# hasindu2008/cornetto

Measured on AMD Instinct MI355X. Metric: Gbases/s scanned (telowin+sdust+boringbits), higher is better.
Workload: dtype u8/u16 integer

## Files before the change

cornetto_amd/csrc/common.hpp:

```cpp
#pragma once
#include <hip/hip_runtime.h>

#include <cstdarg>
#include <cstdint>
#include <cstdio>
#include <cstdlib>
#include <cstring>
#include <algorithm>
#include <atomic>
#include <string>
#include <utility>
#include <vector>

#include "../../include/cornetto_accel.h"

#ifndef CN_STREAM_PRIO
#define CN_STREAM_PRIO 3
#endif

inline std::atomic<uint64_t> cn_uid_counter{1};

struct cornetto_accel {
    int device = 0;
    std::string tf_lut_key;
// ... 23 lines not shown
    int sd_slots = 0;
    int sd_cus = 0;
    int sift_per_cu = 0;
    int sift_per_cu_default = -1;
    int lazy = 0;
    hipStream_t copy_stream = nullptr;
    hipEvent_t ev_cp = nullptr;
    bool copies_pending = false;
    volatile int boost = 0;
    volatile unsigned long long launch_seq = 0;
    hipEvent_t ev3 = nullptr;
    int share = 100;
    int sd_stats = 0;
    struct SdPend {
        int state = 0;
        const void *a = nullptr;
        int32_t T = 0, W = 0;
        void *of = nullptr;
        size_t m_cap = 0, n_cap = 0, cap = 0;
        int64_t key = 0, n_done = 0;
        bool walk_pending = false;
    } sd_pend;
    unsigned long long sd_last[256] = {0};
    uint32_t scan_epoch = 0, scan_tickets = 0;
    uint32_t st_epoch = 0, st_tickets = 0;
    int timing = 2;
};

static inline void *cn_ws(cornetto_accel_t *h, int slot, size_t bytes)
{
    cornetto_accel::Ws &w = h->dev[slot];
    if (bytes == 0) bytes = 16;
    if (w.bytes >= bytes) return w.p;
#ifdef CN_WS_ASYNC
    if (w.p) (void)hipFreeAsync(w.p, h->stream);
    w.p = nullptr;
    w.bytes = 0;
    const size_t want = bytes + bytes / 8;
    if (hipMallocAsync(&w.p, want, h->stream) == hipSuccess) w.bytes = want;
    else w.p = nullptr;
    return w.p;
#else
    if (w.p) (void)hipFree(w.p);
    w.p = nullptr;
    w.bytes = 0;
    const size_t want = bytes + bytes / 8;
// ... 292 lines not shown
```

cornetto_amd/csrc/ivlmerge.hpp:

```cpp
#pragma once
#include "common.hpp"
#include "scan.hpp"

namespace cnivl {
namespace {

constexpr int ST_THREADS = 256, ST_ITEMS = 4, ST_TILE = ST_THREADS * ST_ITEMS;

__device__ __forceinline__ unsigned long long st_shfl_up(unsigned long long v, int d)
{
    return ((unsigned long long)(unsigned)__shfl_up((int)(v >> 32), d) << 32) | (unsigned)__shfl_up((int)v, d);
}

__global__ __launch_bounds__(ST_THREADS) void st_local(const cornetto_ivl_t *v, int64_t n, unsigned long long *kprev, unsigned long long *tile_max)
{
    __shared__ unsigned long long wmax[ST_THREADS / 64];
    const int t = threadIdx.x, lane = t & 63, wv = t >> 6;
    const int64_t j0 = (int64_t)blockIdx.x * ST_TILE + (int64_t)t * ST_ITEMS;
    unsigned long long k[ST_ITEMS], run = 0;
#pragma unroll
    for (int i = 0; i < ST_ITEMS; ++i) {
        k[i] = 0;
        if (j0 + i < n) k[i] = ((unsigned long long)(unsigned)v[j0 + i].ctg << 32) | (unsigned)v[j0 + i].finish;
        run = k[i] > run ? k[i] : run;
// ... 63 lines not shown
__global__ void st_emit(const cornetto_ivl_t *v, int64_t n, const unsigned long long *kinc, const uint32_t *head, const uint32_t *rank, cornetto_ivl_t *out)
{
    const int64_t j = (int64_t)blockIdx.x * blockDim.x + threadIdx.x;
    if (j >= n) return;
    const uint32_t hd = head[j];
    const uint32_t g = rank[j] + hd - 1u;
    if (hd) {
        out[g].ctg = v[j].ctg;
        out[g].start = v[j].start;
    }
    if (j == n - 1 || head[j + 1]) out[g].finish = (int32_t)(kinc[j] & 0xFFFFFFFFull);
}

struct StArgs {
    const cornetto_ivl_t *v;
    const unsigned long long *d_n;
    int64_t n_cap;
    int32_t dist;
    unsigned long long *st;
    uint32_t *ticket;
    uint32_t ticket_base, epoch;
    cornetto_ivl_t *out;
    unsigned long long *d_count;
};

__device__ __forceinline__ unsigned long long st_wave_max(unsigned long long v)
{
#pragma unroll
    for (int d = 32; d >= 1; d >>= 1) {
        const unsigned long long o = ((unsigned long long)(unsigned)__shfl_xor((int)(v >> 32), d) << 32) | (unsigned)__shfl_xor((int)v, d);
        v = o > v ? o : v;
    }
    return v;
}

__global__ __launch_bounds__(ST_THREADS) void st_fused(StArgs A)
{
    __shared__ unsigned long long wmax[ST_THREADS / 64];
    __shared__ uint32_t wcnt[ST_THREADS / 64];
    __shared__ unsigned long long s_in;
    __shared__ uint32_t s_tile, s_base;
    const int t = threadIdx.x, lane = t & 63, wv = t >> 6;
    if (t == 0) s_tile = atomicAdd(A.ticket, 1u) - A.ticket_base;
    __syncthreads();
    const int64_t tile = s_tile;
    if (tile >= (A.n_cap + ST_TILE - 1) / ST_TILE) return;
    const int64_t n = (int64_t)__hip_atomic_load(A.d_n, __ATOMIC_RELAXED, __HIP_MEMORY_SCOPE_AGENT);
    if (n > A.n_cap) return;
    if (tile * ST_TILE >= n) return;
    const int64_t j0 = tile * ST_TILE + (int64_t)t * ST_ITEMS;
    cornetto_ivl_t x[ST_ITEMS + 1];
    unsigned long long k[ST_ITEMS], run = 0;
#pragma unroll
    for (int i = 0; i <= ST_ITEMS; ++i) {
        x[i] = cornetto_ivl_t{0, 0, 0};
        if (j0 + i < n) x[i] = A.v[j0 + i];
    }
#pragma unroll
    for (int i = 0; i < ST_ITEMS; ++i) {
        k[i] = j0 + i < n ? ((unsigned long long)(unsigned)x[i].ctg << 32) | (unsigned)x[i].finish : 0ull;
        run = k[i] > run ? k[i] : run;
    }
    unsigned long long inc = run;
#pragma unroll
    for (int d = 1; d < 64; d <<= 1) {
        const unsigned long long o = st_shfl_up(inc, d);
        if (lane >= d && o > inc) inc = o;
    }
    if (lane == 63) wmax[wv] = inc;
    __syncthreads();
// ... 79 lines not shown
                for (;;) {
                    c = idx >= 0 ? __hip_atomic_load(&st[4 * idx + 3], __ATOMIC_RELAXED, __HIP_MEMORY_SCOPE_AGENT) : ((2ull << 62) | ctag);
                    const bool ready = (c >> 62) != 0 && (c & (0x3FFFFFFFull << 32)) == ctag;
                    if (__builtin_amdgcn_ballot_w64(!ready) == 0) break;
                    __builtin_amdgcn_s_sleep(1);
                }
                const unsigned long long incl = __builtin_amdgcn_ballot_w64((c >> 62) == 2);
                const uint32_t val = (uint32_t)c;
                if (incl) {
                    const int first = __builtin_ctzll(incl);
                    excl += cnscan::wave_sum(lane <= first ? val : 0u);
                    break;
                }
                excl += cnscan::wave_sum(val);
            }
        }
        if (lane == 0) {
            __hip_atomic_store(&st[4 * tile + 3], (2ull << 62) | ctag | (excl + tcnt), __ATOMIC_RELAXED, __HIP_MEMORY_SCOPE_AGENT);
            s_base = excl;
            if (tile == (n - 1) / ST_TILE && A.d_count) *A.d_count = (unsigned long long)excl + tcnt;
        }
    }
    __syncthreads();
    uint32_t rank = s_base + pre;
#pragma unroll
    for (int i = 0; i < ST_ITEMS; ++i) {
        if (j0 + i >= n) break;
        const uint32_t g = rank + hd[i] - 1u;
        if (hd[i]) {
            A.out[g].ctg = x[i].ctg;
            A.out[g].start = x[i].start;
        }
        if (j0 + i == n - 1 || hd[i + 1]) A.out[g].finish = (int32_t)(kinc[i] & 0xFFFFFFFFull);
        rank += hd[i];
    }
}

static inline int merge_fused(cornetto_accel_t *h, const char *name, const cornetto_ivl_t *d_in, const unsigned long long *d_n, int64_t n_cap, int32_t dist,
                              cornetto_ivl_t *d_out, unsigned long long *d_count)
{
    if (n_cap <= 0) return CORNETTO_OK;
    const int64_t nt = (n_cap + ST_TILE - 1) / ST_TILE;
    const size_t need = 64 + (size_t)nt * 32;
    const bool fresh = h->dev[WS_STITCH].bytes < need;
    uint8_t *ws = (uint8_t *)cn_ws(h, WS_STITCH, need);
    if (!ws) return cn_fail(h, CORNETTO_E_NOMEM, "merge: workspace allocation failed");
    const int rc = [&]() -> int {
        if (fresh) {
            CN_HIP(h, hipMemsetAsync(ws, 0, h->dev[WS_STITCH].bytes, h->stream));
            h->st_tickets = 0;
            h->st_epoch = 0;
        }
        uint32_t epoch = (h->st_epoch + 1) & 0x3FFFFFFFu;
        if (epoch == 0) epoch = 1;
        StArgs A{d_in, d_n, n_cap, dist, reinterpret_cast<unsigned long long *>(ws + 64), reinterpret_cast<uint32_t *>(ws), h->st_tickets, epoch, d_out, d_count};
        CN_LAUNCH(h, name, st_fused<<<dim3((unsigned)nt), dim3(ST_THREADS), 0, h->stream>>>(A));
        h->st_epoch = epoch;
        h->st_tickets += (uint32_t)nt;
        return CORNETTO_OK;
    }();
    if (rc != CORNETTO_OK) h->dev[WS_STITCH].bytes = 0;
    return rc;
}

static inline size_t ws_bytes(size_t n)
{
    const size_t nt = (n + ST_TILE - 1) / ST_TILE;
    return n * 16 + (nt + 1) * 8 + ((n + 4095) / 4096 + 1) * 4 + 64;
}

static inline int merge(cornetto_accel_t *h, const char *name, const cornetto_ivl_t *d_in, int64_t n_in, int32_t dist, uint8_t *ws,
                        cornetto_ivl_t *d_out, unsigned long long *d_count)
{
    if (n_in <= 0) return CORNETTO_OK;
    const size_t n = (size_t)n_in, nt = (n + ST_TILE - 1) / ST_TILE;
    unsigned long long *d_k = (unsigned long long *)ws, *d_tile = d_k + n;
    uint32_t *d_head = (uint32_t *)(d_tile + nt + 1), *d_rank = d_head + n, *d_hp = d_rank + n;
    const unsigned nbn = (unsigned)((n + 255) / 256);
// ... 11 lines not shown
```

cornetto_amd/csrc/scan.hpp:

```cpp
#pragma once
#include "common.hpp"

namespace cnscan {
namespace {

constexpr int SC_THREADS = 256;
constexpr int SC_ITEMS = 16;
constexpr int SC_TILE = SC_THREADS * SC_ITEMS;

__device__ __forceinline__ uint32_t wave_incl(uint32_t v, int lane)
{
#pragma unroll
    for (int d = 1; d < 64; d <<= 1) {
        uint32_t o = __shfl_up(v, d);
        if (lane >= d) v += o;
    }
    return v;
}

__global__ __launch_bounds__(SC_THREADS) void scan_local(const uint32_t *in, int64_t n, int stride, uint32_t *out, uint32_t *partial)
{
    __shared__ uint32_t wtot[SC_THREADS / 64];
    const int t = threadIdx.x, lane = t & 63, wv = t >> 6;
    const int64_t base = (int64_t)blockIdx.x * SC_TILE + (int64_t)t * SC_ITEMS;
// ... 123 lines not shown
        const int64_t i = base + k;
        if (i < n) out[i] += add;
    }
}

struct LbArgs {
    const uint32_t *in;
    int64_t n, np;
    int stride, m;
    Outs4 outs;
    unsigned long long *state;
    uint32_t *ticket;
    uint32_t ticket_base, epoch;
    unsigned long long *total;
};

__device__ __forceinline__ uint32_t wave_sum(uint32_t v)
{
#pragma unroll
    for (int d = 32; d >= 1; d >>= 1) v += __shfl_xor(v, d);
    return v;
}

__global__ __launch_bounds__(SC_THREADS) void scan_lookback(LbArgs A)
{
    __shared__ uint32_t wtot[SC_THREADS / 64];
    __shared__ uint32_t s_gid, s_excl;
    const int t = threadIdx.x, lane = t & 63, wv = t >> 6;
    if (t == 0) s_gid = atomicAdd(A.ticket, 1u) - A.ticket_base;
    __syncthreads();
    const int64_t gid = s_gid;
    if (gid >= (int64_t)A.m * A.np) return;
    const int q = (int)(gid / A.np);
    const int64_t tile = gid - (int64_t)q * A.np;
    const int64_t base = tile * SC_TILE + (int64_t)t * SC_ITEMS;
    uint32_t *const out = A.outs.o[q];
    uint32_t v[SC_ITEMS], s = 0;
#pragma unroll
    for (int k = 0; k < SC_ITEMS; ++k) {
        const int64_t i = base + k;
        v[k] = i < A.n ? A.in[i * A.stride + q] : 0u;
        s += v[k];
    }
    const uint32_t inc = wave_incl(s, lane);
    if (lane == 63) wtot[wv] = inc;
    __syncthreads();
    uint32_t pre = inc - s, bt = 0;
#pragma unroll
    for (int w = 0; w < SC_THREADS / 64; ++w) {
        if (w < wv) pre += wtot[w];
        bt += wtot[w];
    }
    if (wv == 0) {
        unsigned long long *const st = A.state + (int64_t)q * A.np;
        const unsigned long long tag = (unsigned long long)(A.epoch & 0x3FFFFFFFu) << 32;
        uint32_t excl = 0;
        if (tile > 0) {
            if (lane == 0) __hip_atomic_store(&st[tile], (1ull << 62) | tag | bt, __ATOMIC_RELAXED, __HIP_MEMORY_SCOPE_AGENT);
            for (int64_t pos = tile - 1;; pos -= 64) {
                const int64_t idx = pos - lane;
                unsigned long long x;
                for (;;) {
                    x = idx >= 0 ? __hip_atomic_load(&st[idx], __ATOMIC_RELAXED, __HIP_MEMORY_SCOPE_AGENT) : ((2ull << 62) | tag);
                    const bool ready = (x >> 62) != 0 && (x & (0x3FFFFFFFull << 32)) == tag;
                    if (__builtin_amdgcn_ballot_w64(!ready) == 0) break;
                    __builtin_amdgcn_s_sleep(1);
                }
                const unsigned long long incl = __builtin_amdgcn_ballot_w64((x >> 62) == 2);
                uint32_t val = (uint32_t)x;
                if (incl) {
                    const int first = __builtin_ctzll(incl);
                    excl += wave_sum(lane <= first ? val : 0u);
                    break;
                }
                excl += wave_sum(val);
            }
        }
        if (lane == 0) {
            __hip_atomic_store(&st[tile], (2ull << 62) | tag | (excl + bt), __ATOMIC_RELAXED, __HIP_MEMORY_SCOPE_AGENT);
            s_excl = excl;
            if (A.total && tile == A.np - 1) A.total[q] = (unsigned long long)excl + bt;
        }
    }
    __syncthreads();
    pre += s_excl;
#pragma unroll
    for (int k = 0; k < SC_ITEMS; ++k) {
        const int64_t i = base + k;
        if (i < A.n) out[i] = pre;
        pre += v[k];
    }
}

static inline int scan_mode()
{
    static const int mode = CN_DEV_INT("CORNETTO_SCAN", 1);
    return mode;
}

static inline int lookback_launch(cornetto_accel_t *h, const char *name, const uint32_t *in, int64_t n, int stride, int m, const Outs4 &o,
                                  unsigned long long *d_total)
{
    const int64_t np = (n + SC_TILE - 1) / SC_TILE;
    const size_t need = 64 + (size_t)m * (size_t)np * 8;
    const bool fresh = h->dev[WS_SCAN].bytes < need;
    uint8_t *ws = (uint8_t *)cn_ws(h, WS_SCAN, need);
    if (!ws) return cn_fail(h, CORNETTO_E_NOMEM, "scan: workspace allocation failed");
    const int rc = [&]() -> int {
        if (fresh) {
            CN_HIP(h, hipMemsetAsync(ws, 0, h->dev[WS_SCAN].bytes, h->stream));
            h->scan_tickets = 0;
            h->scan_epoch = 0;
        }
        uint32_t epoch = (h->scan_epoch + 1) & 0x3FFFFFFFu;
        if (epoch == 0) epoch = 1;
        LbArgs A{in, n, np, stride, m, o, reinterpret_cast<unsigned long long *>(ws + 64), reinterpret_cast<uint32_t *>(ws), h->scan_tickets, epoch, d_total};
        CN_LAUNCH(h, name, scan_lookback<<<dim3((unsigned)(m * np)), dim3(SC_THREADS), 0, h->stream>>>(A));
        h->scan_epoch = epoch;
        h->scan_tickets += (uint32_t)(m * np);
        return CORNETTO_OK;
    }();
    if (rc != CORNETTO_OK) h->dev[WS_SCAN].bytes = 0;
    return rc;
}

static inline int exclusive_u32_multi(cornetto_accel_t *h, const char *name, const uint32_t *in, int64_t n, int stride, int m, uint32_t *const *outs,
                                      uint32_t *partial, unsigned long long *d_total)
{
    if (n <= 0 || m <= 0) return CORNETTO_OK;
    const int64_t np = (n + SC_TILE - 1) / SC_TILE;
    Outs4 o{};
    for (int q = 0; q < m && q < 4; ++q) o.o[q] = outs[q];
    if (scan_mode() != 3) return lookback_launch(h, name, in, n, stride, m < 4 ? m : 4, o, d_total);
    CN_LAUNCH(h, name, scan_local_m<<<dim3((unsigned)np, (unsigned)m), dim3(SC_THREADS), 0, h->stream>>>(in, n, stride, o, partial, np));
    CN_LAUNCH(h, name, scan_partials_m<<<dim3((unsigned)m), dim3(1024), 0, h->stream>>>(partial, np, d_total));
    CN_LAUNCH(h, name, scan_add_m<<<dim3((unsigned)np, (unsigned)m), dim3(SC_THREADS), 0, h->stream>>>(o, n, partial, np));
    return CORNETTO_OK;
}

static inline int exclusive_u32(cornetto_accel_t *h, const char *name, const uint32_t *in, int64_t n, int stride, uint32_t *out,
                                uint32_t *partial, unsigned long long *d_total)
{
    if (n <= 0) return CORNETTO_OK;
    if (scan_mode() != 3) {
        Outs4 o{};
// ... 13 lines not shown
```

cornetto_amd/csrc/sdust.hip:

```cpp
#include <algorithm>
#include <type_traits>
#include <ctime>
#include <sched.h>

#include "common.hpp"
#include "scan.hpp"
#include "tiles.hpp"
#include "ivlmerge.hpp"

namespace {

__device__ __forceinline__ int nt4_code(uint32_t c);
struct SdArgs;
struct SdChunk;
template <bool LEAN = false>
__device__ int sd_find_start(const SdArgs &A, const SdChunk ch, const uint8_t *seq);

struct SdChunk {
    int32_t ctg, start, end;
};
struct SdChunkFill {
    SdChunk *out;
    const int32_t *len;
    int32_t chunk;
// ... 1283 lines not shown
    const uint32_t j = j0 < Lm ? (uint32_t)ps.turn[j0 % ps.P] * stripe_m + j0 / ps.P
                               : ps.P * stripe_m + (j0 - Lm);
    if (dense_list) {
        if (flag[c]) {
            dense_list[r] = (uint32_t)c;
            claim[c] = 1u;
            return;
        }
        perm[j] = (uint32_t)c;
        return;
    }
    uint32_t S = H ? (uint32_t)n_chunks / H : 64u;
    S = S > 64u ? 64u : (S < 1u ? 1u : S);
    uint32_t pos;
    if (flag[c]) {
        pos = r * S;
    } else {
        if (S > 1u && j < H * (S - 1u)) pos = (j / (S - 1u)) * S + 1u + j % (S - 1u);
        else pos = H * S + (j - H * (S - 1u));
    }
    perm[pos] = (uint32_t)c;
}

__global__ void sdust_gather(const uint2 *in, const uint32_t *cnt, const uint32_t *dst_off, uint32_t cap, const SdChunk *chunks,
                             int32_t n_chunks, cornetto_ivl_t *dst, uint32_t dst_cap = 0xFFFFFFFFu)
{
    const int cid = blockIdx.x * blockDim.x + threadIdx.x;
    if (cid >= n_chunks) return;
    uint32_t n = cnt[cid];
    if (n == 0) return;
    if (n > cap) n = cap;
    const int32_t ctg = chunks[cid].ctg;
    const uint2 *src = in + (size_t)cid * cap;
    const uint32_t o = dst_off[cid];
    for (uint32_t i = 0; i < n && o + i < dst_cap; ++i) dst[o + i] = cornetto_ivl_t{ctg, (int32_t)src[i].x, (int32_t)src[i].y};
}

__global__ void sd_sample_count(const uint8_t *bases, const int64_t *ctg_off, const int32_t *ctg_len, unsigned long long *count)
{
    const int c = blockIdx.y;
    const int len = ctg_len[c];
    const uint8_t *seq = bases + ctg_off[c];
    unsigned n = 0;
    for (long long s = (long long)blockIdx.x * blockDim.x + threadIdx.x; s * 2048 + 64 <= len; s += (long long)gridDim.x * blockDim.x)
        n += sd_sample_heavy(SdChunk{c, (int32_t)(s * 2048), (int32_t)std::min<long long>(len, s * 2048 + 2048)}, seq);
    const unsigned long long m = sd_ballot(n != 0);
    (void)m;
    for (int d = 32; d > 0; d >>= 1) n += __shfl_down(n, d);
    if ((threadIdx.x & 63) == 0 && n) atomicAdd(count, (unsigned long long)n);
}

__global__ void sd_make_order(const uint32_t *walk, const uint32_t *iswalk, const uint32_t *rank, int32_t n_chunks, uint32_t *order)
{
    const int k = blockIdx.x * blockDim.x + threadIdx.x;
    if (k >= n_chunks) return;
    const uint32_t nw = walk[0];
    if ((uint32_t)k < nw) order[k] = walk[2 + k];
    if (!iswalk[k]) order[nw + (uint32_t)k - rank[k]] = (uint32_t)k;
}

}

extern "C" {

}

namespace {
int sd_one_go_finish(cornetto_accel_t *h, cornetto_asm_t *a, cornetto_ivl_t *of, unsigned long long *p_tot, size_t cap, size_t n_cap, size_t m_cap, int64_t key,
                     bool walk_pending, cornetto_ivl_t **ivls, int64_t *n_ivls)
{
    if (hipStreamSynchronize(h->stream) != hipSuccess) {
        cornetto_free(of);
        return cn_fail(h, CORNETTO_E_HIP, "sdust: stitch / copy back failed");
    }
    const uint32_t ovf_f = (uint32_t)(p_tot[1] & 0xFFFFFFFFull);
    const bool wtab_f = (p_tot[1] >> 32) != 0;
    const unsigned long long rows_f = p_tot[0], out_f = rows_f ? p_tot[9] : 0ull;
    if (!wtab_f && ovf_f <= cap && rows_f <= n_cap && out_f != ~0ull && out_f <= m_cap && out_f <= rows_f && (rows_f == 0 || out_f > 0)) {
        if (walk_pending) a->sd_walk_key = key;
        a->sd_est_rows = (int64_t)rows_f;
        a->sd_est_out = (int64_t)out_f;
        cn_timing_end(h);
        *ivls = of;
        *n_ivls = (int64_t)out_f;
        return 0;
    }
    cornetto_free(of);
    a->sd_est_key = -1;
    return 1;
}

int sdust_asm_impl(cornetto_accel_t *h, const cornetto_asm_t *a_in, int32_t T, int32_t W, cornetto_ivl_t **ivls, int64_t *n_ivls, const int phase)
{
    static const bool trace = CN_DEV_INT("CORNETTO_SDUST_TRACE", 0) != 0;
    struct timespec ts0;
    clock_gettime(CLOCK_MONOTONIC, &ts0);
    auto stamp = [&](const char *what) {
        if (!trace) return;
        struct timespec t;
        clock_gettime(CLOCK_MONOTONIC, &t);
        fprintf(stderr, "[sdust trace] %-22s %8.3f ms\n", what, (t.tv_sec - ts0.tv_sec) * 1e3 + (t.tv_nsec - ts0.tv_nsec) * 1e-6);
    };
    if (!h || !a_in || !ivls || !n_ivls) return cn_fail(h, CORNETTO_E_ARG, "sdust: bad argument");
    cornetto_asm_t *a = const_cast<cornetto_asm_t *>(a_in);
    *ivls = nullptr;
    *n_ivls = 0;
    if (W < 3 || W > 1026) return cn_fail(h, CORNETTO_E_UNSUPPORTED, "sdust: -w %d outside 3..1026 (the reference crashes below 3)", W);
    if (T < 0 || T > (1 << 20)) return cn_fail(h, CORNETTO_E_UNSUPPORTED, "sdust: -t %d outside 0..2^20", T);
    CN_HIP(h, hipSetDevice(h->device));
    cn_timing_begin(h);
// ... 23 lines not shown
        h->sd_cus = cus;
    }
    stamp("kernel attributes");
    const int64_t sd_waves = w64_path ? CN_DEV_INT("CORNETTO_SDUST_WAVES", std::max(1, h->sd_slots / h->sd_cus * h->share / 100) * h->sd_cus) : 0;

    int64_t chunk = CN_DEV_INT("CORNETTO_SDUST_CHUNK", 0);
    if (chunk <= 0) {
        chunk = 1536;
        const int64_t lanes = sd_waves * 64;
        if (lanes > 0 && a->total / lanes >= 1536) {
            const int64_t rounds = a->total / (lanes * 1536);
            chunk = std::min<int64_t>(3072, ((a->total + lanes * rounds - 1) / (lanes * rounds) + 63) / 64 * 64);
        }
    }
    chunk = std::max<int64_t>(16, chunk);
    if (W > 257 && CN_DEV_INT("CORNETTO_SDUST_CHUNK", 0) <= 0) chunk = std::max<int64_t>(chunk, 32 * (int64_t)W);
    const int sift_env = CN_DEV_INT("CORNETTO_SDUST_SIFT", 1);
    if (w64_path && sift_env < 0 && a->sd_auto < 0) {
        if (a->n > 4096 || a->total < 2000000000ll) {
            a->sd_auto = 1;
        } else {
            unsigned long long *d_cnt8 = (unsigned long long *)cn_ws(h, WS_SD_STATS, 2048 + 64 * 64);
            unsigned long long *p_cnt8 = (unsigned long long *)cn_pin(h, PIN_SMALL, 2048);
            if (!d_cnt8 || !p_cnt8) return cn_fail(h, CORNETTO_E_NOMEM, "sdust: workspace allocation failed");
            CN_HIP(h, hipMemsetAsync(d_cnt8, 0, 8, h->stream));
            int32_t maxlen = 0;
            for (int32_t c = 0; c < a->n; ++c) maxlen = std::max(maxlen, a->len[c]);
            const unsigned bx = (unsigned)std::min<int64_t>(64, std::max<int64_t>(1, (maxlen / 2048 + 255) / 256));
            sd_sample_count<<<dim3(bx, (unsigned)a->n), dim3(256), 0, h->stream>>>(a->d_bases, a->d_off, a->d_len, d_cnt8);
            CN_HIP(h, hipGetLastError());
            CN_HIP(h, hipMemcpyAsync(p_cnt8 + 220, d_cnt8, 8, hipMemcpyDeviceToHost, h->stream));
            CN_HIP(h, hipStreamSynchronize(h->stream));
            const int64_t samples = a->total / 2048, heavy = (int64_t)p_cnt8[220];
            a->sd_auto = heavy * 256 >= std::max<int64_t>(samples, 1) && heavy >= 64 ? 1 : 0;
            if (trace) fprintf(stderr, "[sdust trace] %lld of %lld samples inside repeat arrays: %s\n", (long long)heavy, (long long)samples, a->sd_auto ? "sift / resolve" : "per-lane recurrence");
        }
    }
    bool sift_on = w64_path && (sift_env > 0 || (sift_env < 0 && a->sd_auto == 1));
    if (sift_on && CN_DEV_INT("CORNETTO_SDUST_CHUNK", 0) <= 0) chunk = SIFT_CHUNK_DEFAULT;
    if (sift_on && (chunk % 64 != 0 || chunk < 256 || chunk > 3968)) sift_on = false;
    const int tail_pct = sift_on ? 0 : std::min(90, std::max(0, CN_DEV_INT("CORNETTO_SDUST_TAIL", 0)));
    const int tail_div = std::min(16, std::max(1, CN_DEV_INT("CORNETTO_SDUST_TAILDIV", 4)));
    const int64_t small = std::max<int64_t>(64, (chunk / tail_div + 63) / 64 * 64);
    const int64_t tail_from = tail_pct > 0 && tail_div > 1 ? a->total - a->total * tail_pct / 100 : a->total + 1;
    const int64_t key = chunk + (int64_t)tail_pct * (1ll << 40) + (int64_t)tail_div * (1ll << 48) + (sift_on ? 1ll << 56 : 0);
    if (a->sd_chunk != key && tail_pct == 0) {
// ... 82 lines not shown
            }
        }
    }
    const size_t nc = (size_t)a->sd_n_chunks;
    cornetto_ivl_t *o = nullptr;
    int64_t n_out = 0;
    stamp("chunk table");
    if (nc > 0) {
        const SdChunk *d_chunks = reinterpret_cast<const SdChunk *>(a->d_sd_chunks);
        uint32_t *d_cnt = (uint32_t *)cn_ws(h, WS_SD_CNT, nc * 8 + ((nc + 4095) / 4096 + 1) * 4);
        unsigned long long *d_tot = (unsigned long long *)cn_ws(h, WS_SD_STATS, 2048 + 64 * 64);
        unsigned long long *p_tot = (unsigned long long *)cn_pin(h, PIN_SMALL, 2048);
        if (!d_cnt || !d_tot || !p_tot) return cn_fail(h, CORNETTO_E_NOMEM, "sdust: workspace allocation failed");
        uint32_t *d_off = d_cnt + nc, *d_part = d_off + nc;
        stamp("small workspaces");
        const bool env_stats = CN_DEV_INT("CORNETTO_SDUST_STATS", 0) != 0;
        const bool want_stats = env_stats || h->sd_stats != 0;
        size_t cap = (size_t)std::max<int64_t>(16, chunk / 32);
        cap = (size_t)CN_DEV_INT("CORNETTO_SDUST_CAP", (int)cap);
        if (h->dev[WS_SD_OUT].bytes / (nc * sizeof(uint2)) > cap) cap = h->dev[WS_SD_OUT].bytes / (nc * sizeof(uint2));
        unsigned long long tot = 0;
        uint2 *d_out = nullptr;
        const int64_t est_key = key * 131 + T * 1031 + W;
        const bool one_go = w64_path && sift_on && !want_stats && a->sd_est_key == est_key && a->sd_est_rows >= 0 && CN_DEV_INT("CORNETTO_SDUST_FUSED", 1);
        if (phase == 1 && !one_go)
            return CORNETTO_OK;
        for (int attempt = 0; attempt < 4; ++attempt) {
            d_out = (uint2 *)cn_ws(h, WS_SD_OUT, nc * cap * sizeof(uint2));
            if (!d_out) return cn_fail(h, CORNETTO_E_NOMEM, "sdust: workspace allocation of %zu bytes failed", nc * cap * sizeof(uint2));
            CN_HIP(h, hipMemsetAsync(d_tot, 0, 2048 + 64 * 64, h->stream));
            uint32_t *d_slots = (uint32_t *)cn_ws(h, WS_SD_OFF, (size_t)(std::max<int64_t>(sd_waves, 1) + SD_WPB) * 64 * 64 * sizeof(uint32_t));
            if (!d_slots) return cn_fail(h, CORNETTO_E_NOMEM, "sdust: workspace allocation failed");
            stamp("row + slot workspaces");
            const bool use_w64 = w64_path;
            SdArgs A{a->d_bases, a->d_off, a->d_len, d_chunks, (int32_t)nc, T, W, d_out, d_cnt, (uint32_t)cap,
                     want_stats ? d_tot + 2 : nullptr, reinterpret_cast<uint32_t *>(d_tot + 1), d_slots, nullptr,
                     reinterpret_cast<uint32_t *>(d_tot + 8), nullptr, 0, CN_DEV_INT("CORNETTO_SDUST_RUNON", 1), (int32_t)chunk, a->d_wtab, a->d_wtab_base, reinterpret_cast<uint32_t *>(d_tot + 1) + 1};
            unsigned nb = (unsigned)((nc + 63) / 64);
            bool sift_walk_pending = false;
            bool dense_pending = false;
            struct DenseJoin {
                cornetto_accel_t *h;
                bool *pending;
                ~DenseJoin() { if (*pending && h->stream2) (void)hipStreamSynchronize(h->stream2); }
            } dense_join{h, &dense_pending};
            if (use_w64 && sift_on) {
                CN_HIP(h, hipMemsetAsync(d_cnt, 0, nc * 4, h->stream));
                const uint32_t reg_cap = (uint32_t)(chunk + 128);
                const uint32_t lds_wave = sift_lds_bytes(reg_cap);
                int lmin = 1;
                while (5 * (lmin + 1) <= T && lmin < 16) ++lmin;
                const bool walk_known = a->d_sd_walk && a->sd_walk_key == key;
                const size_t walk_words = 2 + 4 * nc + ((nc + 4095) / 4096 + 2);
                if (!walk_known) {
                    if (a->d_sd_walk) { (void)hipFree(a->d_sd_walk); a->d_sd_walk = nullptr; }
                    a->sd_walk_key = -1;
                    if (cn_obj_malloc(h, (void **)&a->d_sd_walk, walk_words * 4) != hipSuccess) return cn_fail(h, CORNETTO_E_NOMEM, "sdust: device allocation failed");
                    CN_HIP(h, hipMemsetAsync(a->d_sd_walk, 0, (2 + 2 * nc) * 4, h->stream));
                }
                uint32_t *d_wflag = a->d_sd_walk + 2 + nc, *d_wrank = d_wflag + nc, *d_worder = d_wrank + nc, *d_wpart = d_worder + nc;
                SiftArgs S{a->d_bases, a->d_off, a->d_len, d_chunks, (int32_t)nc, T, W, lds_wave, reg_cap,
                           walk_known ? d_worder : nullptr, walk_known ? nullptr : a->d_sd_walk, walk_known ? nullptr : d_wflag,
                           reinterpret_cast<uint32_t *>(d_tot + 256), T / 10 + 1, lmin, CN_DEV_INT("CORNETTO_SIFT_ABL", 0),
                           std::min(65, std::max(1, CN_DEV_INT("CORNETTO_SIFT_DP", 24))), std::min(65, std::max(1, CN_DEV_INT("CORNETTO_SIFT_L2SKIP", 48)))};
                sift_walk_pending = !walk_known;
                SdArgs R = A;
                R.stats = want_stats ? d_tot + 200 : nullptr;
                const bool cap_default = reg_cap == SIFT_CAP_DEFAULT && !CN_DEV_INT("CORNETTO_SIFT_GENERIC", 0) && !CN_DEV_INT("CORNETTO_SIFT_ABL", 0);
                if (h->sift_per_cu == 0 || h->sift_per_cu_default != (cap_default ? 1 : 0)) {
                    int per_cu = 0;
// ... 144 lines not shown
                if ((unsigned)sd_waves < nb) nb = (unsigned)sd_waves;
                nb = (nb + SD_WPB - 1) / SD_WPB * SD_WPB;
                if (want_stats) CN_LAUNCH(h, "sdust_kernel", sdust_w64<true><<<dim3(nb / SD_WPB), dim3(64 * SD_WPB), 0, h->stream>>>(A));
                else CN_LAUNCH(h, "sdust_kernel", sdust_w64<false><<<dim3(nb / SD_WPB), dim3(64 * SD_WPB), 0, h->stream>>>(A));
            } else if (W - 2 <= 64) {
                CN_LAUNCH(h, "sdust_kernel", sdust_kernel<64><<<dim3(nb), dim3(64), 0, h->stream>>>(A));
            } else if (W - 2 <= 255) {
                CN_LAUNCH(h, "sdust_kernel", sdust_kernel<256><<<dim3(nb), dim3(64), 0, h->stream>>>(A));
            } else {
                int rc = 512;
                while (rc < W - 2) rc <<= 1;
                const size_t NL = (size_t)nb * 64;
                uint8_t *g = (uint8_t *)cn_ws(h, WS_SD_OFF, NL * ((size_t)rc * 5 + 512) + 64);
                if (!g) return cn_fail(h, CORNETTO_E_NOMEM, "sdust: workspace allocation of %zu bytes failed", NL * ((size_t)rc * 5 + 512));
                uint32_t *g_cw = reinterpret_cast<uint32_t *>(g), *g_cv = g_cw + 64 * NL, *g_slot = g_cv + 64 * NL;
                uint8_t *g_ring = reinterpret_cast<uint8_t *>(g_slot + (size_t)rc * NL);
                CN_LAUNCH(h, "sdust_kernel", sdust_kernel_g<<<dim3(nb), dim3(64), 0, h->stream>>>(A, g_ring, g_cw, g_cv, g_slot, rc));
            }
            if (!sift_on) __atomic_fetch_add(&h->launch_seq, 1ull, __ATOMIC_RELEASE);
            if (dense_pending) {
                CN_HIP(h, hipStreamWaitEvent(h->stream, h->ev2, 0));
                dense_pending = false;
            }
            CN_TRY(cnscan::exclusive_u32(h, "sdust_scan", d_cnt, (int64_t)nc, 1, d_off, d_part, d_tot));
            if (one_go) {
                size_t n_cap = (size_t)(a->sd_est_rows + a->sd_est_rows / 8 + 4096);
                if (CN_DEV_INT("CORNETTO_SDUST_EST_FORCE", 0) > 0) n_cap = (size_t)CN_DEV_INT("CORNETTO_SDUST_EST_FORCE", 0);
                const size_t m_cap = (size_t)(a->sd_est_out + a->sd_est_out / 16 + 1024);
                uint8_t *ws = (uint8_t *)cn_ws(h, WS_SD_DST, 2 * n_cap * sizeof(cornetto_ivl_t) + cnivl::ws_bytes(n_cap));
                cornetto_ivl_t *of = (cornetto_ivl_t *)cn_result_alloc(std::max<size_t>(m_cap * sizeof(cornetto_ivl_t), (size_t)1 << 20));
                if (ws && of && n_cap < 0x7fffffffull) {
                    cornetto_ivl_t *d_dst = (cornetto_ivl_t *)(ws + cnivl::ws_bytes(n_cap)), *d_st = d_dst + n_cap;
                    const unsigned nbg = (unsigned)((nc + 255) / 256);
                    CN_LAUNCH(h, "sdust_gather", sdust_gather<<<dim3(nbg), dim3(256), 0, h->stream>>>(d_out, d_cnt, d_off, (uint32_t)cap, d_chunks, (int32_t)nc, d_dst, (uint32_t)n_cap));
                    CN_HIP(h, hipMemsetAsync(d_tot + 9, 0xFF, 8, h->stream));
                    int rcf = cnivl::merge_fused(h, "sdust_stitch", d_dst, d_tot, (int64_t)n_cap, 0, d_st, d_tot + 9);
                    if (rcf != CORNETTO_OK) { cornetto_free(of); return rcf; }
                    stamp("tail queued");
                    if (hipMemcpyAsync(of, d_st, m_cap * sizeof(cornetto_ivl_t), hipMemcpyDeviceToHost, h->stream) != hipSuccess ||
                        hipMemcpyAsync(p_tot, d_tot, 128, hipMemcpyDeviceToHost, h->stream) != hipSuccess) {
                        (void)hipStreamSynchronize(h->stream);
                        cornetto_free(of);
                        return cn_fail(h, CORNETTO_E_HIP, "sdust: stitch / copy back failed");
                    }
                    if (phase == 1) {
                        h->sd_pend.state = 1; h->sd_pend.a = a; h->sd_pend.T = T; h->sd_pend.W = W; h->sd_pend.of = of;
                        h->sd_pend.m_cap = m_cap; h->sd_pend.n_cap = n_cap; h->sd_pend.cap = cap; h->sd_pend.key = key; h->sd_pend.walk_pending = sift_walk_pending;
                        return CORNETTO_OK;
                    }
                    const int fin = sd_one_go_finish(h, a, of, p_tot, cap, n_cap, m_cap, key, sift_walk_pending, ivls, n_ivls);
                    if (fin <= 0) {
                        if (fin == 0) stamp("results on the host (one go)");
                        return fin;
                    }
                } else if (of) {
                    cornetto_free(of);
                }
            }
            stamp("main kernel queued");
            CN_HIP(h, hipMemcpyAsync(p_tot, d_tot, want_stats ? 2048 : 128, hipMemcpyDeviceToHost, h->stream));
            CN_HIP(h, hipStreamSynchronize(h->stream));
            stamp("main kernel done");
            if (want_stats) {
                memcpy(h->sd_last, p_tot, 2048);
                if (a->sd_flagged >= 0) h->sd_last[7] = (unsigned long long)a->sd_flagged;
                h->sd_last[254] = nb;
                h->sd_last[255] = nc;
            }
            if (env_stats)
                for (int b = 0; b < 32; ++b)
                    if (p_tot[16 + 4 * b])
                        fprintf(stderr, "[sdust stats]   waves that ran %4.1f-%4.1f ms: %6llu, job fetches %llu, find_perfect calls %llu (%llu with candidates)\n", b * 0.5, b * 0.5 + 0.5,
                                p_tot[16 + 4 * b], p_tot[18 + 4 * b], p_tot[19 + 4 * b], p_tot[17 + 4 * b]);
            if (env_stats && sift_on)
                fprintf(stderr, "[sdust stats] sift: tiles %llu, positions with ct > T/10 %llu, after L1 %llu, after L2 %llu; resolve: steps %llu, window reads %llu (behind a gap of 2 / 3-4 / 5-8: %llu / %llu / %llu), dp tiles %llu; passes with candidates %llu; base-by-base steps of chunks with other bytes %llu\n",
                        p_tot[206], p_tot[203], p_tot[204], p_tot[205], p_tot[200], p_tot[201], p_tot[209], p_tot[210], p_tot[211], p_tot[208], p_tot[202], p_tot[207]);
            if (env_stats)
                fprintf(stderr, "[sdust stats] flagged low-complexity %llu; chunks %zu waves %u wave-steps %llu find_perfect calls %llu (%llu with candidates) plain groups %llu; wave time avg %.1f us max %.1f us; queue: %.1f fetch rounds and %.1f us per wave\n", p_tot[7], nc, nb,
                        p_tot[2], p_tot[3], p_tot[10], p_tot[4], nb ? (double)p_tot[5] / nb / 100.0 : 0.0, (double)p_tot[6] / 100.0, nb ? (double)p_tot[11] / nb : 0.0, nb ? (double)p_tot[12] / nb / 100.0 : 0.0);
            const uint32_t ovf = (uint32_t)(p_tot[1] & 0xFFFFFFFFull);
            const bool need_wtab = (p_tot[1] >> 32) != 0;
// ... 17 lines not shown
                (void)hipFree(d_wcnt);
                if (rc != CORNETTO_OK) return rc;
                if (e != hipSuccess) return cn_fail(h, CORNETTO_E_HIP, "sdust: word-count table build failed");
                continue;
            }
            if (sift_walk_pending && !need_wtab) a->sd_walk_key = key;
            if (ovf <= cap) {
                tot = p_tot[0];
                break;
            }
            if (attempt >= 2) return cn_fail(h, CORNETTO_E_HIP, "sdust: a chunk produced %u intervals after resizing to %zu", ovf, cap);
            cap = ovf;
        }
        if (tot > 0x7fffffffull) return cn_fail(h, CORNETTO_E_UNSUPPORTED, "sdust: %llu intervals", tot);
        o = (cornetto_ivl_t *)cn_result_alloc((tot ? tot : 1) * sizeof(cornetto_ivl_t));
        if (!o) return cn_fail(h, CORNETTO_E_NOMEM, "sdust: host allocation failed");
        stamp("result buffer");
        if (tot > 0) {
            const size_t n = (size_t)tot;
            uint8_t *ws = (uint8_t *)cn_ws(h, WS_SD_DST, 2 * n * sizeof(cornetto_ivl_t) + cnivl::ws_bytes(n));
            if (!ws) { cornetto_free(o); return cn_fail(h, CORNETTO_E_NOMEM, "sdust: workspace allocation failed"); }
            cornetto_ivl_t *d_dst = (cornetto_ivl_t *)(ws + cnivl::ws_bytes(n)), *d_st = d_dst + n;
            const unsigned nbg = (unsigned)((nc + 255) / 256);
            CN_LAUNCH(h, "sdust_gather", sdust_gather<<<dim3(nbg), dim3(256), 0, h->stream>>>(d_out, d_cnt, d_off, (uint32_t)cap, d_chunks, (int32_t)nc, d_dst));
            CN_TRY(cnivl::merge(h, "sdust_stitch", d_dst, (int64_t)n, 0, ws, d_st, d_tot + 9));
            stamp("gather+stitch queued");
            if (trace) { (void)hipStreamSynchronize(h->stream); stamp("gather+stitch done (trace only)"); }
            if (hipMemcpyAsync(o, d_st, n * sizeof(cornetto_ivl_t), hipMemcpyDeviceToHost, h->stream) != hipSuccess ||
                hipMemcpyAsync(p_tot, d_tot + 9, 8, hipMemcpyDeviceToHost, h->stream) != hipSuccess ||
                hipStreamSynchronize(h->stream) != hipSuccess) {
                cornetto_free(o);
                return cn_fail(h, CORNETTO_E_HIP, "sdust: stitch / copy back failed");
            }
            n_out = (int64_t)p_tot[0];
            stamp("results on the host");
        }
        if (sift_on) {
            a->sd_est_key = est_key;
            a->sd_est_rows = (int64_t)tot;
            a->sd_est_out = n_out;
        }
    }
    cn_timing_end(h);
    if (!o) {
        o = (cornetto_ivl_t *)malloc(sizeof(cornetto_ivl_t));
        if (!o) return cn_fail(h, CORNETTO_E_NOMEM, "sdust: host allocation failed");
    }
// ... 132 lines not shown
```

Measured before the change: 493.9.

## Fuse sdust scan into gather and write stitched results directly to host memory

```diff
diff --git a/cornetto_amd/csrc/common.hpp b/cornetto_amd/csrc/common.hpp
--- a/cornetto_amd/csrc/common.hpp
+++ b/cornetto_amd/csrc/common.hpp
@@ -69,6 +69,10 @@
         bool walk_pending = false;
     } sd_pend;
     unsigned long long sd_last[256] = {0};
+    struct SdClean {
+        const void *cnt = nullptr, *tot = nullptr;
+        size_t nc = 0;
+    } sd_clean;
     uint32_t scan_epoch = 0, scan_tickets = 0;
     uint32_t st_epoch = 0, st_tickets = 0;
     int timing = 2;
diff --git a/cornetto_amd/csrc/ivlmerge.hpp b/cornetto_amd/csrc/ivlmerge.hpp
--- a/cornetto_amd/csrc/ivlmerge.hpp
+++ b/cornetto_amd/csrc/ivlmerge.hpp
@@ -109,6 +109,8 @@
     uint32_t ticket_base, epoch;
     cornetto_ivl_t *out;
     unsigned long long *d_count;
+    unsigned long long *h_tot;
+    const unsigned long long *d_word1;
 };
 
 __device__ __forceinline__ unsigned long long st_wave_max(unsigned long long v)
@@ -126,13 +128,22 @@
     __shared__ unsigned long long wmax[ST_THREADS / 64];
     __shared__ uint32_t wcnt[ST_THREADS / 64];
     __shared__ unsigned long long s_in;
-    __shared__ uint32_t s_tile, s_base;
+    __shared__ uint32_t s_tile, s_base, s_closed;
+    __shared__ uint32_t s_out[3 * ST_TILE];
     const int t = threadIdx.x, lane = t & 63, wv = t >> 6;
-    if (t == 0) s_tile = atomicAdd(A.ticket, 1u) - A.ticket_base;
+    if (t == 0) {
+        s_tile = atomicAdd(A.ticket, 1u) - A.ticket_base;
+        s_closed = 0;
+    }
     __syncthreads();
     const int64_t tile = s_tile;
     if (tile >= (A.n_cap + ST_TILE - 1) / ST_TILE) return;
     const int64_t n = (int64_t)__hip_atomic_load(A.d_n, __ATOMIC_RELAXED, __HIP_MEMORY_SCOPE_AGENT);
+    if (A.h_tot && tile == 0 && t == 0) {
+        A.h_tot[0] = (unsigned long long)n;
+        A.h_tot[1] = *A.d_word1;
+        __builtin_amdgcn_fence(__ATOMIC_RELEASE, "");
+    }
     if (n > A.n_cap) return;
     if (tile * ST_TILE >= n) return;
     const int64_t j0 = tile * ST_TILE + (int64_t)t * ST_ITEMS;
@@ -258,22 +269,36 @@
         }
     }
     __syncthreads();
-    uint32_t rank = s_base + pre;
+    const uint32_t base = s_base;
+    uint32_t l = pre;
 #pragma unroll
     for (int i = 0; i < ST_ITEMS; ++i) {
         if (j0 + i >= n) break;
-        const uint32_t g = rank + hd[i] - 1u;
+        const uint32_t g = l + hd[i] - 1u;
         if (hd[i]) {
-            A.out[g].ctg = x[i].ctg;
-            A.out[g].start = x[i].start;
-        }
-        if (j0 + i == n - 1 || hd[i + 1]) A.out[g].finish = (int32_t)(kinc[i] & 0xFFFFFFFFull);
-        rank += hd[i];
-    }
+            s_out[3 * g] = (uint32_t)x[i].ctg;
+            s_out[3 * g + 1] = (uint32_t)x[i].start;
+        }
+        if (j0 + i == n - 1 || hd[i + 1]) {
+            const uint32_t fin = (uint32_t)(kinc[i] & 0xFFFFFFFFull);
+            if (g == 0xFFFFFFFFu) {
+                A.out[base - 1u].finish = (int32_t)fin;
+            } else {
+                s_out[3 * g + 2] = fin;
+                if (g + 1u == tcnt) s_closed = 1;
+            }
+        }
+        l += hd[i];
+    }
+    __syncthreads();
+    const uint32_t words = 3u * tcnt - (s_closed ? 0u : 1u);
+    uint32_t *const ow = reinterpret_cast<uint32_t *>(A.out + base);
+    for (uint32_t d = t; tcnt && d < words; d += ST_THREADS) ow[d] = s_out[d];
+    if (A.h_tot) __builtin_amdgcn_fence(__ATOMIC_RELEASE, "");
 }
 
 static inline int merge_fused(cornetto_accel_t *h, const char *name, const cornetto_ivl_t *d_in, const unsigned long long *d_n, int64_t n_cap, int32_t dist,
-                              cornetto_ivl_t *d_out, unsigned long long *d_count)
+                              cornetto_ivl_t *d_out, unsigned long long *d_count, unsigned long long *h_tot = nullptr, const unsigned long long *d_word1 = nullptr)
 {
     if (n_cap <= 0) return CORNETTO_OK;
     const int64_t nt = (n_cap + ST_TILE - 1) / ST_TILE;
@@ -289,7 +314,7 @@
         }
         uint32_t epoch = (h->st_epoch + 1) & 0x3FFFFFFFu;
         if (epoch == 0) epoch = 1;
-        StArgs A{d_in, d_n, n_cap, dist, reinterpret_cast<unsigned long long *>(ws + 64), reinterpret_cast<uint32_t *>(ws), h->st_tickets, epoch, d_out, d_count};
+        StArgs A{d_in, d_n, n_cap, dist, reinterpret_cast<unsigned long long *>(ws + 64), reinterpret_cast<uint32_t *>(ws), h->st_tickets, epoch, d_out, d_count, h_tot, d_word1};
         CN_LAUNCH(h, name, st_fused<<<dim3((unsigned)nt), dim3(ST_THREADS), 0, h->stream>>>(A));
         h->st_epoch = epoch;
         h->st_tickets += (uint32_t)nt;
diff --git a/cornetto_amd/csrc/scan.hpp b/cornetto_amd/csrc/scan.hpp
--- a/cornetto_amd/csrc/scan.hpp
+++ b/cornetto_amd/csrc/scan.hpp
@@ -169,6 +169,34 @@
     return v;
 }
 
+__device__ __forceinline__ uint32_t lookback_excl(unsigned long long *st, int64_t tile, unsigned long long tag, uint32_t bt, int lane)
+{
+    uint32_t excl = 0;
+    if (tile > 0) {
+        if (lane == 0) __hip_atomic_store(&st[tile], (1ull << 62) | tag | bt, __ATOMIC_RELAXED, __HIP_MEMORY_SCOPE_AGENT);
+        for (int64_t pos = tile - 1;; pos -= 64) {
+            const int64_t idx = pos - lane;
+            unsigned long long x;
+            for (;;) {
+                x = idx >= 0 ? __hip_atomic_load(&st[idx], __ATOMIC_RELAXED, __HIP_MEMORY_SCOPE_AGENT) : ((2ull << 62) | tag);
+                const bool ready = (x >> 62) != 0 && (x & (0x3FFFFFFFull << 32)) == tag;
+                if (__builtin_amdgcn_ballot_w64(!ready) == 0) break;
+                __builtin_amdgcn_s_sleep(1);
+            }
+            const unsigned long long incl = __builtin_amdgcn_ballot_w64((x >> 62) == 2);
+            uint32_t val = (uint32_t)x;
+            if (incl) {
+                const int first = __builtin_ctzll(incl);
+                excl += wave_sum(lane <= first ? val : 0u);
+                break;
+            }
+            excl += wave_sum(val);
+        }
+    }
+    if (lane == 0) __hip_atomic_store(&st[tile], (2ull << 62) | tag | (excl + bt), __ATOMIC_RELAXED, __HIP_MEMORY_SCOPE_AGENT);
+    return excl;
+}
+
 __global__ __launch_bounds__(SC_THREADS) void scan_lookback(LbArgs A)
 {
     __shared__ uint32_t wtot[SC_THREADS / 64];
@@ -201,30 +229,8 @@
     if (wv == 0) {
         unsigned long long *const st = A.state + (int64_t)q * A.np;
         const unsigned long long tag = (unsigned long long)(A.epoch & 0x3FFFFFFFu) << 32;
-        uint32_t excl = 0;
-        if (tile > 0) {
-            if (lane == 0) __hip_atomic_store(&st[tile], (1ull << 62) | tag | bt, __ATOMIC_RELAXED, __HIP_MEMORY_SCOPE_AGENT);
-            for (int64_t pos = tile - 1;; pos -= 64) {
-                const int64_t idx = pos - lane;
-                unsigned long long x;
-                for (;;) {
-                    x = idx >= 0 ? __hip_atomic_load(&st[idx], __ATOMIC_RELAXED, __HIP_MEMORY_SCOPE_AGENT) : ((2ull << 62) | tag);
-                    const bool ready = (x >> 62) != 0 && (x & (0x3FFFFFFFull << 32)) == tag;
-                    if (__builtin_amdgcn_ballot_w64(!ready) == 0) break;
-                    __builtin_amdgcn_s_sleep(1);
-                }
-                const unsigned long long incl = __builtin_amdgcn_ballot_w64((x >> 62) == 2);
-                uint32_t val = (uint32_t)x;
-                if (incl) {
-                    const int first = __builtin_ctzll(incl);
-                    excl += wave_sum(lane <= first ? val : 0u);
-                    break;
-                }
-                excl += wave_sum(val);
-            }
-        }
+        const uint32_t excl = lookback_excl(st, tile, tag, bt, lane);
         if (lane == 0) {
-            __hip_atomic_store(&st[tile], (2ull << 62) | tag | (excl + bt), __ATOMIC_RELAXED, __HIP_MEMORY_SCOPE_AGENT);
             s_excl = excl;
             if (A.total && tile == A.np - 1) A.total[q] = (unsigned long long)excl + bt;
         }
@@ -245,29 +251,50 @@
     return mode;
 }
 
-static inline int lookback_launch(cornetto_accel_t *h, const char *name, const uint32_t *in, int64_t n, int stride, int m, const Outs4 &o,
-                                  unsigned long long *d_total)
-{
-    const int64_t np = (n + SC_TILE - 1) / SC_TILE;
-    const size_t need = 64 + (size_t)m * (size_t)np * 8;
+struct LbSlot {
+    unsigned long long *state;
+    uint32_t *ticket;
+    uint32_t ticket_base, epoch;
+};
+static inline int lookback_reserve(cornetto_accel_t *h, size_t tiles, LbSlot *s)
+{
+    const size_t need = 64 + tiles * 8;
     const bool fresh = h->dev[WS_SCAN].bytes < need;
     uint8_t *ws = (uint8_t *)cn_ws(h, WS_SCAN, need);
     if (!ws) return cn_fail(h, CORNETTO_E_NOMEM, "scan: workspace allocation failed");
+    if (fresh) {
+        if (hipMemsetAsync(ws, 0, h->dev[WS_SCAN].bytes, h->stream) != hipSuccess) {
+            h->dev[WS_SCAN].bytes = 0;
+            return cn_fail(h, CORNETTO_E_HIP, "scan: clearing the tile states failed");
+        }
+        h->scan_tickets = 0;
+        h->scan_epoch = 0;
+    }
+    uint32_t epoch = (h->scan_epoch + 1) & 0x3FFFFFFFu;
+    if (epoch == 0) epoch = 1;
+    *s = LbSlot{reinterpret_cast<unsigned long long *>(ws + 64), reinterpret_cast<uint32_t *>(ws), h->scan_tickets, epoch};
+    return CORNETTO_OK;
+}
+static inline void lookback_commit(cornetto_accel_t *h, const LbSlot &s, size_t tiles)
+{
+    h->scan_epoch = s.epoch;
+    h->scan_tickets += (uint32_t)tiles;
+}
+static inline void lookback_reset(cornetto_accel_t *h) { h->dev[WS_SCAN].bytes = 0; }
+
+static inline int lookback_launch(cornetto_accel_t *h, const char *name, const uint32_t *in, int64_t n, int stride, int m, const Outs4 &o,
+                                  unsigned long long *d_total)
+{
+    const int64_t np = (n + SC_TILE - 1) / SC_TILE;
+    LbSlot s;
+    CN_TRY(lookback_reserve(h, (size_t)m * (size_t)np, &s));
     const int rc = [&]() -> int {
-        if (fresh) {
-            CN_HIP(h, hipMemsetAsync(ws, 0, h->dev[WS_SCAN].bytes, h->stream));
-            h->scan_tickets = 0;
-            h->scan_epoch = 0;
-        }
-        uint32_t epoch = (h->scan_epoch + 1) & 0x3FFFFFFFu;
-        if (epoch == 0) epoch = 1;
-        LbArgs A{in, n, np, stride, m, o, reinterpret_cast<unsigned long long *>(ws + 64), reinterpret_cast<uint32_t *>(ws), h->scan_tickets, epoch, d_total};
+        LbArgs A{in, n, np, stride, m, o, s.state, s.ticket, s.ticket_base, s.epoch, d_total};
         CN_LAUNCH(h, name, scan_lookback<<<dim3((unsigned)(m * np)), dim3(SC_THREADS), 0, h->stream>>>(A));
-        h->scan_epoch = epoch;
-        h->scan_tickets += (uint32_t)(m * np);
+        lookback_commit(h, s, (size_t)m * (size_t)np);
         return CORNETTO_OK;
     }();
-    if (rc != CORNETTO_OK) h->dev[WS_SCAN].bytes = 0;
+    if (rc != CORNETTO_OK) lookback_reset(h);
     return rc;
 }
 
diff --git a/cornetto_amd/csrc/sdust.hip b/cornetto_amd/csrc/sdust.hip
--- a/cornetto_amd/csrc/sdust.hip
+++ b/cornetto_amd/csrc/sdust.hip
@@ -1329,7 +1329,7 @@
     perm[pos] = (uint32_t)c;
 }
 
-__global__ void sdust_gather(const uint2 *in, const uint32_t *cnt, const uint32_t *dst_off, uint32_t cap, const SdChunk *chunks,
+__global__ void sdust_gather_off(const uint2 *in, const uint32_t *cnt, const uint32_t *dst_off, uint32_t cap, const SdChunk *chunks,
                              int32_t n_chunks, cornetto_ivl_t *dst, uint32_t dst_cap = 0xFFFFFFFFu)
 {
     const int cid = blockIdx.x * blockDim.x + threadIdx.x;
@@ -1341,6 +1341,66 @@
     const uint2 *src = in + (size_t)cid * cap;
     const uint32_t o = dst_off[cid];
     for (uint32_t i = 0; i < n && o + i < dst_cap; ++i) dst[o + i] = cornetto_ivl_t{ctg, (int32_t)src[i].x, (int32_t)src[i].y};
+}
+
+struct SdGatherArgs {
+    const uint2 *in;
+    uint32_t *cnt;
+    uint32_t cap;
+    const SdChunk *chunks;
+    int32_t n_chunks;
+    cornetto_ivl_t *dst;
+    uint32_t dst_cap;
+    unsigned long long *state;
+    uint32_t *ticket;
+    uint32_t ticket_base, epoch;
+    unsigned long long *tot;
+    int32_t leave_clean;
+};
+constexpr int SD_GATHER_THREADS = 256;
+__global__ __launch_bounds__(SD_GATHER_THREADS) void sdust_gather(SdGatherArgs A)
+{
+    __shared__ uint32_t wtot[SD_GATHER_THREADS / 64];
+    __shared__ uint32_t s_tile, s_excl;
+    const int t = threadIdx.x, lane = t & 63, wv = t >> 6;
+    if (t == 0) s_tile = atomicAdd(A.ticket, 1u) - A.ticket_base;
+    __syncthreads();
+    const int64_t tile = s_tile, np = ((int64_t)A.n_chunks + SD_GATHER_THREADS - 1) / SD_GATHER_THREADS;
+    if (tile >= np) return;
+    const int64_t cid = tile * SD_GATHER_THREADS + t;
+    const uint32_t raw = cid < A.n_chunks ? A.cnt[cid] : 0u;
+    const uint32_t inc = cnscan::wave_incl(raw, lane);
+    if (lane == 63) wtot[wv] = inc;
+    __syncthreads();
+    uint32_t pre = inc - raw, bt = 0;
+#pragma unroll
+    for (int w = 0; w < SD_GATHER_THREADS / 64; ++w) {
+        if (w < wv) pre += wtot[w];
+        bt += wtot[w];
+    }
+    if (wv == 0) {
+        const uint32_t excl = cnscan::lookback_excl(A.state, tile, (unsigned long long)(A.epoch & 0x3FFFFFFFu) << 32, bt, lane);
+        if (lane == 0) {
+            s_excl = excl;
+            if (tile == np - 1) A.tot[0] = (unsigned long long)excl + bt;
+        }
+    }
+    if (A.leave_clean && tile == np - 1) {
+        if (t == 0) {
+            A.tot[10] = A.tot[1];
+            A.tot[1] = 0;
+            A.tot[8] = 0;
+        }
+        for (int k = 256 + t; k < 768; k += SD_GATHER_THREADS) A.tot[k] = 0;
+    }
+    __syncthreads();
+    if (raw == 0) return;
+    if (A.leave_clean) A.cnt[cid] = 0;
+    const uint32_t n = raw > A.cap ? A.cap : raw;
+    const int32_t ctg = A.chunks[cid].ctg;
+    const uint2 *src = A.in + (size_t)cid * A.cap;
+    const uint32_t o = s_excl + pre;
+    for (uint32_t i = 0; i < n && o + i < A.dst_cap; ++i) A.dst[o + i] = cornetto_ivl_t{ctg, (int32_t)src[i].x, (int32_t)src[i].y};
 }
 
 __global__ void sd_sample_count(const uint8_t *bases, const int64_t *ctg_off, const int32_t *ctg_len, unsigned long long *count)
@@ -1378,6 +1438,7 @@
 {
     if (hipStreamSynchronize(h->stream) != hipSuccess) {
         cornetto_free(of);
+        h->sd_clean = cornetto_accel::SdClean{};
         return cn_fail(h, CORNETTO_E_HIP, "sdust: stitch / copy back failed");
     }
     const uint32_t ovf_f = (uint32_t)(p_tot[1] & 0xFFFFFFFFull);
@@ -1393,6 +1454,7 @@
         return 0;
     }
     cornetto_free(of);
+    h->sd_clean = cornetto_accel::SdClean{};
     a->sd_est_key = -1;
     return 1;
 }
@@ -1462,6 +1524,7 @@
         } else {
             unsigned long long *d_cnt8 = (unsigned long long *)cn_ws(h, WS_SD_STATS, 2048 + 64 * 64);
             unsigned long long *p_cnt8 = (unsigned long long *)cn_pin(h, PIN_SMALL, 2048);
+            h->sd_clean = cornetto_accel::SdClean{};
             if (!d_cnt8 || !p_cnt8) return cn_fail(h, CORNETTO_E_NOMEM, "sdust: workspace allocation failed");
             CN_HIP(h, hipMemsetAsync(d_cnt8, 0, 8, h->stream));
             int32_t maxlen = 0;
@@ -1590,13 +1653,15 @@
         unsigned long long tot = 0;
         uint2 *d_out = nullptr;
         const int64_t est_key = key * 131 + T * 1031 + W;
-        const bool one_go = w64_path && sift_on && !want_stats && a->sd_est_key == est_key && a->sd_est_rows >= 0 && CN_DEV_INT("CORNETTO_SDUST_FUSED", 1);
+        bool one_go = w64_path && sift_on && !want_stats && a->sd_est_key == est_key && a->sd_est_rows >= 0 && CN_DEV_INT("CORNETTO_SDUST_FUSED", 1);
         if (phase == 1 && !one_go)
             return CORNETTO_OK;
         for (int attempt = 0; attempt < 4; ++attempt) {
             d_out = (uint2 *)cn_ws(h, WS_SD_OUT, nc * cap * sizeof(uint2));
             if (!d_out) return cn_fail(h, CORNETTO_E_NOMEM, "sdust: workspace allocation of %zu bytes failed", nc * cap * sizeof(uint2));
-            CN_HIP(h, hipMemsetAsync(d_tot, 0, 2048 + 64 * 64, h->stream));
+            const bool ws_clean = one_go && h->sd_clean.cnt == d_cnt && h->sd_clean.tot == d_tot && h->sd_clean.nc == nc && CN_DEV_INT("CORNETTO_SDUST_KEEPCLEAN", 1);
+            h->sd_clean = cornetto_accel::SdClean{};
+            if (!ws_clean) CN_HIP(h, hipMemsetAsync(d_tot, 0, 2048 + 64 * 64, h->stream));
             uint32_t *d_slots = (uint32_t *)cn_ws(h, WS_SD_OFF, (size_t)(std::max<int64_t>(sd_waves, 1) + SD_WPB) * 64 * 64 * sizeof(uint32_t));
             if (!d_slots) return cn_fail(h, CORNETTO_E_NOMEM, "sdust: workspace allocation failed");
             stamp("row + slot workspaces");
@@ -1613,7 +1678,7 @@
                 ~DenseJoin() { if (*pending && h->stream2) (void)hipStreamSynchronize(h->stream2); }
             } dense_join{h, &dense_pending};
             if (use_w64 && sift_on) {
-                CN_HIP(h, hipMemsetAsync(d_cnt, 0, nc * 4, h->stream));
+                if (!ws_clean) CN_HIP(h, hipMemsetAsync(d_cnt, 0, nc * 4, h->stream));
                 const uint32_t reg_cap = (uint32_t)(chunk + 128);
                 const uint32_t lds_wave = sift_lds_bytes(reg_cap);
                 int lmin = 1;
@@ -1804,27 +1869,50 @@
                 CN_HIP(h, hipStreamWaitEvent(h->stream, h->ev2, 0));
                 dense_pending = false;
             }
-            CN_TRY(cnscan::exclusive_u32(h, "sdust_scan", d_cnt, (int64_t)nc, 1, d_off, d_part, d_tot));
             if (one_go) {
                 size_t n_cap = (size_t)(a->sd_est_rows + a->sd_est_rows / 8 + 4096);
                 if (CN_DEV_INT("CORNETTO_SDUST_EST_FORCE", 0) > 0) n_cap = (size_t)CN_DEV_INT("CORNETTO_SDUST_EST_FORCE", 0);
                 const size_t m_cap = (size_t)(a->sd_est_out + a->sd_est_out / 16 + 1024);
                 uint8_t *ws = (uint8_t *)cn_ws(h, WS_SD_DST, 2 * n_cap * sizeof(cornetto_ivl_t) + cnivl::ws_bytes(n_cap));
                 cornetto_ivl_t *of = (cornetto_ivl_t *)cn_result_alloc(std::max<size_t>(m_cap * sizeof(cornetto_ivl_t), (size_t)1 << 20));
+                bool miss = false;
                 if (ws && of && n_cap < 0x7fffffffull) {
                     cornetto_ivl_t *d_dst = (cornetto_ivl_t *)(ws + cnivl::ws_bytes(n_cap)), *d_st = d_dst + n_cap;
-                    const unsigned nbg = (unsigned)((nc + 255) / 256);
-                    CN_LAUNCH(h, "sdust_gather", sdust_gather<<<dim3(nbg), dim3(256), 0, h->stream>>>(d_out, d_cnt, d_off, (uint32_t)cap, d_chunks, (int32_t)nc, d_dst, (uint32_t)n_cap));
-                    CN_HIP(h, hipMemsetAsync(d_tot + 9, 0xFF, 8, h->stream));
-                    int rcf = cnivl::merge_fused(h, "sdust_stitch", d_dst, d_tot, (int64_t)n_cap, 0, d_st, d_tot + 9);
+                    void *of_dev = nullptr, *tot_dev = nullptr;
+                    const bool deliver = CN_DEV_INT("CORNETTO_SDUST_DELIVER", 1) && hipHostGetDevicePointer(&of_dev, of, 0) == hipSuccess && of_dev &&
+                                         hipHostGetDevicePointer(&tot_dev, p_tot, 0) == hipSuccess && tot_dev;
+                    if (!deliver) (void)hipGetLastError();
+                    const size_t ntg = (nc + SD_GATHER_THREADS - 1) / SD_GATHER_THREADS;
+                    cnscan::LbSlot lb;
+                    int rcf = cnscan::lookback_reserve(h, ntg, &lb);
+                    if (rcf == CORNETTO_OK) {
+                        rcf = [&]() -> int {
+                            SdGatherArgs G{d_out, d_cnt, (uint32_t)cap, d_chunks, (int32_t)nc, d_dst, (uint32_t)n_cap, lb.state, lb.ticket, lb.ticket_base, lb.epoch, d_tot, deliver ? 1 : 0};
+                            CN_LAUNCH(h, "sdust_gather", sdust_gather<<<dim3((unsigned)ntg), dim3(SD_GATHER_THREADS), 0, h->stream>>>(G));
+                            cnscan::lookback_commit(h, lb, ntg);
+                            return CORNETTO_OK;
+                        }();
+                        if (rcf != CORNETTO_OK) cnscan::lookback_reset(h);
+                    }
+                    if (rcf != CORNETTO_OK) { cornetto_free(of); return rcf; }
+                    if (deliver) {
+                        p_tot[0] = ~0ull;
+                        p_tot[9] = ~0ull;
+                        rcf = cnivl::merge_fused(h, "sdust_stitch", d_dst, d_tot, (int64_t)n_cap, 0, (cornetto_ivl_t *)of_dev, (unsigned long long *)tot_dev + 9,
+                                                 (unsigned long long *)tot_dev, d_tot + 10);
+                    } else {
+                        CN_HIP(h, hipMemsetAsync(d_tot + 9, 0xFF, 8, h->stream));
+                        rcf = cnivl::merge_fused(h, "sdust_stitch", d_dst, d_tot, (int64_t)n_cap, 0, d_st, d_tot + 9);
+                    }
                     if (rcf != CORNETTO_OK) { cornetto_free(of); return rcf; }
                     stamp("tail queued");
-                    if (hipMemcpyAsync(of, d_st, m_cap * sizeof(cornetto_ivl_t), hipMemcpyDeviceToHost, h->stream) != hipSuccess ||
-                        hipMemcpyAsync(p_tot, d_tot, 128, hipMemcpyDeviceToHost, h->stream) != hipSuccess) {
+                    if (!deliver && (hipMemcpyAsync(of, d_st, m_cap * sizeof(cornetto_ivl_t), hipMemcpyDeviceToHost, h->stream) != hipSuccess ||
+                                     hipMemcpyAsync(p_tot, d_tot, 128, hipMemcpyDeviceToHost, h->stream) != hipSuccess)) {
                         (void)hipStreamSynchronize(h->stream);
                         cornetto_free(of);
                         return cn_fail(h, CORNETTO_E_HIP, "sdust: stitch / copy back failed");
                     }
+                    if (deliver) h->sd_clean = cornetto_accel::SdClean{d_cnt, d_tot, nc};
                     if (phase == 1) {
                         h->sd_pend.state = 1; h->sd_pend.a = a; h->sd_pend.T = T; h->sd_pend.W = W; h->sd_pend.of = of;
                         h->sd_pend.m_cap = m_cap; h->sd_pend.n_cap = n_cap; h->sd_pend.cap = cap; h->sd_pend.key = key; h->sd_pend.walk_pending = sift_walk_pending;
@@ -1835,10 +1923,17 @@
                         if (fin == 0) stamp("results on the host (one go)");
                         return fin;
                     }
+                    miss = true;
                 } else if (of) {
                     cornetto_free(of);
                 }
-            }
+                one_go = false;
+                if (miss) {
+                    attempt = -1;
+                    continue;
+                }
+            }
+            CN_TRY(cnscan::exclusive_u32(h, "sdust_scan", d_cnt, (int64_t)nc, 1, d_off, d_part, d_tot));
             stamp("main kernel queued");
             CN_HIP(h, hipMemcpyAsync(p_tot, d_tot, want_stats ? 2048 : 128, hipMemcpyDeviceToHost, h->stream));
             CN_HIP(h, hipStreamSynchronize(h->stream));
@@ -1902,7 +1997,7 @@
             if (!ws) { cornetto_free(o); return cn_fail(h, CORNETTO_E_NOMEM, "sdust: workspace allocation failed"); }
             cornetto_ivl_t *d_dst = (cornetto_ivl_t *)(ws + cnivl::ws_bytes(n)), *d_st = d_dst + n;
             const unsigned nbg = (unsigned)((nc + 255) / 256);
-            CN_LAUNCH(h, "sdust_gather", sdust_gather<<<dim3(nbg), dim3(256), 0, h->stream>>>(d_out, d_cnt, d_off, (uint32_t)cap, d_chunks, (int32_t)nc, d_dst));
+            CN_LAUNCH(h, "sdust_gather", sdust_gather_off<<<dim3(nbg), dim3(256), 0, h->stream>>>(d_out, d_cnt, d_off, (uint32_t)cap, d_chunks, (int32_t)nc, d_dst));
             CN_TRY(cnivl::merge(h, "sdust_stitch", d_dst, (int64_t)n, 0, ws, d_st, d_tot + 9));
             stamp("gather+stitch queued");
             if (trace) { (void)hipStreamSynchronize(h->stream); stamp("gather+stitch done (trace only)"); }
```

After: 487.2. -1.4%, worse.
